# lowmee/xchu_slam

Measured on AMD Instinct MI355X. Metric: NDT scans/sec (120k-pt scan vs 200k-voxel localmap, 30 iters) at 1/2/4/8 GPUs; % HBM BW, higher is better.
Workload: dtype f32 (f64 accumulate)

## Files before the change

xchu_slam_amd/csrc/host_sort.hip:

```cpp
#include "ndt_host.h"

namespace ndt::host {

ndt_status scan_ctx(ndt_ctx* c, Lane L, int nb, ScanCtx* sc) {
    sc->tickets = c->opt.tile_tickets ? 1 : 0;
    if ((size_t)nb > L.s.scan_status.cap) {
        TRY(ensure(c, L.s.scan_status, (size_t)nb));
        HIPCHK(c, hipMemsetAsync(L.s.scan_status.p, 0, L.s.scan_status.cap * sizeof(unsigned long long), L.st));
    }
    if (!L.s.scan_ticket.p) {
        TRY(ensure(c, L.s.scan_ticket, 1));
        HIPCHK(c, hipMemsetAsync(L.s.scan_ticket.p, 0, sizeof(unsigned long long), L.st));
        L.s.scan_tickets = 0;
    }
    sc->status = L.s.scan_status.p;
    sc->ticket = L.s.scan_ticket.p;
    sc->ticket_base = L.s.scan_tickets;
    sc->epoch = ++L.s.scan_epoch;
    sc->nb = nb;
    if (sc->tickets) L.s.scan_tickets += (unsigned long long)nb;
    return NDT_OK;
}

ndt_status enqueue_scan(ndt_ctx* c, Lane L, const int* in, int n_host, const int* n_dev, int* out, int* total_out, GridHeader* herr) {
// ... 17 lines not shown
}

int radix_launch_passes(const ndt_ctx* c) {
    if (c->rerun_full) return 4;
    return c->opt.radix_force > 0 ? std::min(c->opt.radix_force, 4) : c->radix_pred;
}
void note_grid_width(ndt_ctx* c, long long cells, int dense) {
    if (cells <= 0) return;
    const long long top = dense ? cells - 1 : cells;
    int bits = 0;
    while (bits < 31 && (top >> bits) != 0) ++bits;
    c->radix_pred = std::min(4, std::max(1, (bits + 1 + 7) / 8));
}

ndt_status enqueue_bin_and_sort(ndt_ctx* c, Lane L, const float4* pts, int n, int dense, GridHeader* h, float leaf, int layout,
                                int binning, int2* cloud_span, int passes) {
    if (&L.s == &c->s && !cloud_span) c->inc_ok = false;
    const int nb_mm = std::max(1, std::min(ceil_div(n, 4 * kBlock), 1024));
    TRY(ensure(c, L.s.mm, (size_t)nb_mm * 7));
    const int items = radix_items(c, n);
    const int nb_sort = std::max(1, ceil_div(n, kBlock * items));
    const size_t n_kv = cloud_span ? (size_t)n + (size_t)n / 4 : (size_t)n;
    TRY(ensure(c, L.s.k0, n_kv)); TRY(ensure(c, L.s.v0, n_kv)); TRY(ensure(c, L.s.k1, n_kv)); TRY(ensure(c, L.s.v1, n_kv));
    TRY(ensure(c, L.s.radix_aux, kRadixAuxWords));
    TRY(ensure(c, L.s.radix_status, radix_status_words(nb_sort)));
    TRY(ensure(c, L.s.seg_start, (size_t)n + 1));
    hipLaunchKernelGGL(k_minmax, dim3(nb_mm), dim3(kBlock), 0, L.st, pts, n, dense, L.s.mm.p, L.s.radix_aux.p,
                       cloud_span ? c->d_clk.p + 3 : nullptr, nullptr, nullptr, nullptr);
    const int nb_keys = std::max(1, std::min(ceil_div(n, 4 * kBlock), 512));
    hipLaunchKernelGGL(k_keys, dim3(nb_keys), dim3(kBlock), 0, L.st, pts, n, dense, L.s.mm.p, nb_mm, h, leaf, c->prm.min_points_per_voxel,
                       c->prm.min_covar_eigvalue_mult, layout, binning, L.s.k0.p, L.s.v0.p, L.s.radix_aux.p, L.s.radix_status.p,
                       (int)radix_status_words(nb_sort), cloud_span ? c->grid.p : nullptr, (long long)c->grid.cap, cloud_span ? c->table.p : nullptr,
                       1LL << c->max_log2cap, nullptr, 0);
    for (int pass = 0; pass < passes; ++pass)
        launch_radix_pass(c, L, items, nb_sort, L.s.k0.p, L.s.v0.p, L.s.k1.p, L.s.v1.p, n, pass, h, h, passes - 1);
    const int nb_seg = std::max(1, ceil_div(n, kTileKeys));
    ScanCtx sc;
    TRY(scan_ctx(c, L, nb_seg, &sc));
    hipLaunchKernelGGL(k_seg_scan, dim3(nb_seg), dim3(kBlock), 0, L.st, L.s.k0.p, L.s.k1.p, n, h, L.s.seg_start.p, sc);
    if (cloud_span) {
        ScanCtx sc2;
        TRY(scan_ctx(c, L, nb_seg, &sc2));
        hipLaunchKernelGGL(k_cloud_scan, dim3(nb_seg), dim3(kBlock), 0, L.st, L.s.seg_start.p, n, h, cloud_span, sc2, c->max_log2cap);
    }
    return NDT_OK;
}

ndt_status enqueue_downsample_finalize(ndt_ctx* c, Lane L, const GridHeader* h, const float4* in, int n, float4* out) {
    TRY(ensure(c, L.s.sorted_pts, std::max(n, 1)));
    const int nb = std::max(1, std::min(ceil_div(n, 4 * kBlock), 2048));
    hipLaunchKernelGGL(k_sorted_gather, dim3(nb), dim3(kBlock), 0, L.st, in, L.s.v0.p, L.s.v1.p, h, L.s.sorted_pts.p, n);
    hipLaunchKernelGGL(k_downsample_finalize, dim3(std::max(1, ceil_div(n, kBlock))), dim3(kBlock), 0, L.st, L.s.sorted_pts.p,
                       L.s.seg_start.p, h, out);
    HIPCHK(c, hipGetLastError());
    return NDT_OK;
}

}
```

xchu_slam_amd/csrc/host_target.hip:

```cpp
#include "ndt_host.h"

namespace ndt::host {

namespace {

ndt_status grow_grid(ndt_ctx* c) {
    const long long want_cells = std::min<long long>(std::max<long long>(2 * c->grid_cells_seen, 16ll << 20), 1ll << 30);
    if ((long long)c->grid.cap < want_cells) TRY(ensure(c, c->grid, (size_t)want_cells));
    return NDT_OK;
}

ndt_status alloc_cloud_buffers(ndt_ctx* c, size_t max_cloud) {
    TRY(ensure(c, c->recs, max_cloud)); TRY(ensure(c, c->cent, max_cloud)); TRY(ensure(c, c->icovd, max_cloud * 9));
    TRY(ensure(c, c->evals, max_cloud * 3)); TRY(ensure(c, c->cloud_key, max_cloud));
    return NDT_OK;
}

constexpr int kFinalize3WavesMaxPoints = 4 << 20;

ndt_status prepare_target_buffers(ndt_ctx* c, int M, int* nb_cloud) {
    TRY(grow_grid(c));
    const size_t max_cloud = std::max(1, M / std::max(1, c->prm.min_points_per_voxel) + 1);
    TRY(alloc_cloud_buffers(c, max_cloud));
    unsigned l = 6;
    while (l < 30 && (1ull << l) < 4ull * max_cloud) ++l;
    c->max_log2cap = l;
    TRY(ensure(c, c->table, (size_t)1 << l));
    *nb_cloud = std::max(1, ceil_div((long long)max_cloud, kBlock));
    TRY(ensure(c, c->s.cloud_span, (size_t)*nb_cloud * kBlock));
    TRY(ensure(c, c->valid_part, max_cloud / 64 + 1));
    return NDT_OK;
}

ndt_status launch_finalize(ndt_ctx* c, int M, int nb_cloud) {
    auto* fin = M < kFinalize3WavesMaxPoints ? k_leaf_finalize<3> : k_leaf_finalize<2>;
    hipLaunchKernelGGL(fin, dim3(nb_cloud), dim3(kBlock), 0, c->stream.get(), c->target_ptr, c->s.k0.p, c->s.k1.p, c->s.v0.p,
                       c->s.v1.p, c->s.cloud_span.p, c->d_hdr.p, c->recs.p, c->cent.p, c->icovd.p, c->cloud_key.p,
                       c->evals.p, c->grid.p, c->table.p, c->valid_part.p);
    HIPCHK(c, hipGetLastError());
    return NDT_OK;
}

ndt_status enqueue_target_build(ndt_ctx* c) {
    c->inc_ok = false;
    ++c->n_builds_full;
    const int M = c->M;
    int nb_cloud = 0;
    TRY(prepare_target_buffers(c, M, &nb_cloud));
    TRY(enqueue_bin_and_sort(c, main_lane(c), c->target_ptr, M, c->target_dense, c->d_hdr.p, c->prm.resolution, 0, c->prm.precision_mode == 2 ? 1 : 0,
                             c->s.cloud_span.p, radix_launch_passes(c)));
    TRY(launch_finalize(c, M, nb_cloud));
    c->inc_ok = c->prm.precision_mode != 2 && c->target_dense == 1 && M > 0;
    return NDT_OK;
}

ndt_status enqueue_target_append(ndt_ctx* c, int n_old, int n_new, const float4* new_src) {
    const int M = n_old + n_new;
    int nb_cloud = 0;
    TRY(prepare_target_buffers(c, M, &nb_cloud));
    Lane Q{c->stream.get(), c->s_inc};
    float4* copy_to = new_src ? const_cast<float4*>(c->target_ptr) + n_old : nullptr;
    const float4* pts_new = new_src ? new_src : c->target_ptr + n_old;
    const int nq = std::max(n_new, 1);
    const int nb_mm = std::max(1, std::min(ceil_div(nq, 4 * kBlock), 1024));
    TRY(ensure(c, Q.s.mm, (size_t)nb_mm * 7));
    const int items = radix_items(c, nq);
    const int nb_sort = std::max(1, ceil_div(nq, kBlock * items));
    TRY(ensure(c, Q.s.k0, nq)); TRY(ensure(c, Q.s.v0, nq)); TRY(ensure(c, Q.s.k1, nq)); TRY(ensure(c, Q.s.v1, nq));
    TRY(ensure(c, Q.s.radix_aux, kRadixAuxWords));
    TRY(ensure(c, Q.s.radix_status, radix_status_words(nb_sort)));
    TRY(ensure(c, c->s.seg_start, (size_t)M + 1));
    hipLaunchKernelGGL(k_minmax, dim3(nb_mm), dim3(kBlock), 0, c->stream.get(), pts_new, n_new, 1, Q.s.mm.p, Q.s.radix_aux.p, c->d_clk.p + 3,
                       c->d_hdr.p, c->d_hdr_prev.p, copy_to);
    if (c->tgt_ev_valid) HIPCHK(c, hipEventRecord(c->ev_tgt.get(), c->stream.get()));
    const long long clear_words = std::max<long long>((long long)c->grid.cap, 2LL << c->max_log2cap) / 4;
    const int nb_keys = std::max(1, (int)std::min<long long>(std::max<long long>(ceil_div(nq, 4 * kBlock), ceil_div(clear_words, 4LL * kBlock)), 512));
    hipLaunchKernelGGL(k_keys, dim3(nb_keys), dim3(kBlock), 0, c->stream.get(), pts_new, n_new, 1, Q.s.mm.p, nb_mm, c->d_hdr.p, c->prm.resolution,
                       c->prm.min_points_per_voxel, c->prm.min_covar_eigvalue_mult, 0, 0, Q.s.k0.p, Q.s.v0.p, Q.s.radix_aux.p,
                       Q.s.radix_status.p, (int)radix_status_words(nb_sort), c->grid.p, (long long)c->grid.cap, c->table.p, 1LL << c->max_log2cap,
                       c->d_hdr_prev.p, n_old);
    const int passes = radix_launch_passes(c);
    for (int pass = 0; pass < passes; ++pass)
        launch_radix_pass(c, Q, items, nb_sort, Q.s.k0.p, Q.s.v0.p, Q.s.k1.p, Q.s.v1.p, n_new, pass, c->d_hdr.p, c->d_hdr.p, passes - 1);
    hipLaunchKernelGGL(k_merge_append, dim3(std::max(1, ceil_div(M, kMergeTileKeys))), dim3(kBlock), 0, c->stream.get(), c->s.k0.p, c->s.v0.p,
                       c->s.k1.p, c->s.v1.p, c->d_hdr_prev.p, n_old, Q.s.k0.p, Q.s.v0.p, Q.s.k1.p, Q.s.v1.p, n_new, c->d_hdr.p,
                       c->target_ptr);
    const Lane L = main_lane(c);
    const int nb_seg = std::max(1, ceil_div(M, kTileKeys));
    ScanCtx sc, sc2;
    TRY(scan_ctx(c, L, nb_seg, &sc));
    hipLaunchKernelGGL(k_seg_scan, dim3(nb_seg), dim3(kBlock), 0, c->stream.get(), c->s.k0.p, c->s.k1.p, M, c->d_hdr.p, c->s.seg_start.p, sc);
    TRY(scan_ctx(c, L, nb_seg, &sc2));
    hipLaunchKernelGGL(k_cloud_scan, dim3(nb_seg), dim3(kBlock), 0, c->stream.get(), c->s.seg_start.p, M, c->d_hdr.p, c->s.cloud_span.p, sc2,
                       c->max_log2cap);
    TRY(launch_finalize(c, M, nb_cloud));
    return NDT_OK;
}

}

ndt_status build_target(ndt_ctx* c) {
    ++c->tgt_gen;
    c->tgt_ev_valid = c->lanes.fit_tgt_used;
    if (c->tgt_ev_valid) HIPCHK(c, hipEventRecord(c->ev_tgt.get(), c->stream.get()));
    TRY(enqueue_target_build(c));
    c->build_unchecked = true;
    c->built_since_align = true;
    c->grid_valid = true;
    c->fit_valid = false;
    c->grid_res = c->prm.resolution;
// ... 202 lines not shown
```

xchu_slam_amd/csrc/ndt_api.hip:

```cpp
#include "ndt_host.h"

static bool valid_params(const ndt_params* p) {
    return p && p->resolution > 0.f && std::isfinite(p->resolution) && p->max_iter >= 0 && p->search >= 0 && p->search <= 3 &&
           p->min_points_per_voxel >= 1 && p->precision_mode >= 0 && p->precision_mode <= 2;
}

static ndt_status create_buffers(ndt_ctx* c) {
    for (DevBuf<GridHeader>* h : {&c->d_hdr, &c->d_hdr_ds, &c->d_hdr_prev, &c->fe.d_hdr, &c->fit_ix.hdr, &c->fe.sor_ix.hdr}) TRY(ensure(c, *h, 1));
    HIPCHK(c, hipMemset(c->fe.d_hdr.p, 0, sizeof(GridHeader)));
    TRY(make_pinned(c, c->h_hdr, 1, hipHostMallocDefault));
    TRY(ensure(c, c->d_state, 1));
    TRY(ensure(c, c->d_state2, 1));
    TRY(make_pinned(c, c->h_state, 1, hipHostMallocCoherent));
    TRY(make_pinned(c, c->h_rb, 8, hipHostMallocCoherent));
    TRY(ensure(c, c->d_clk, 4));
    TRY(ensure(c, c->d_hist, c->hist_cap));
    TRY(ensure(c, c->d_async, 1));
    TRY(make_pinned(c, c->h_async, 1, hipHostMallocDefault));
    TRY(make_event(c, c->ev_tgt, hipEventDisableTiming));
    std::memset(c->h_state.get(), 0, sizeof(AlignState));
    std::memset(c->h_rb.get(), 0, 8 * sizeof(unsigned long long));
    return NDT_OK;
}

// ... 199 lines not shown
```

xchu_slam_amd/csrc/ndt_host.h:

```cpp
#pragma once
#include <hip/hip_runtime.h>
#include <string>
#include <vector>
#include <cstring>
#include <cstdlib>
#include <cstdio>
#include <algorithm>
#include <cmath>
#include <atomic>
#include <condition_variable>
#include <deque>
#include <functional>
#include <memory>
#include <mutex>
#include <shared_mutex>
#include <thread>

#include "../../include/ndt_hip.h"
#include "ndt_kernels.h"

namespace ndt::host {

constexpr int kTileKeys = kBlock * 16;

// ... 211 lines not shown
    Pinned<AsyncOut> h_async;
    SideLanes lanes;
    Scratch s;
    Scratch s_inc;
    DevBuf<GridHeader> d_hdr_prev;
    bool inc_ok = false;
    int radix_pred = 4;
    bool build_unchecked = false;
    bool rerun_full = false;
    float al_guess[16] = {0};
    int al_berr = 0;
    long long n_builds_full = 0, n_builds_merge = 0, n_builds_rerun = 0, n_rerun_lookback = 0;
    unsigned long long tgt_gen = 0, fit_ix_gen = ~0ull, align_tgt_gen = ~0ull;
    DevBuf<VoxelRec> recs;
    DevBuf<float4> cent;
    DevBuf<double> icovd, evals;
    DevBuf<int> cloud_key;
    DevBuf<int> valid_part;
    DevBuf<int2> table;
    unsigned max_log2cap = 6;
    DevBuf<int> grid;
    long long grid_cells_seen = 0;
    DevBuf<float4> source;
    int N = 0;
    bool has_source = false;
    const float4* src_pend = nullptr;
    DevBuf<float4> source_ord;
    DevBuf<int> ord_k0, ord_v0, ord_k1, ord_v1;
    const float4* pass_src = nullptr;
    FrontEnd fe;
    DevBuf<AlignState> d_state;
    DevBuf<AlignState> d_state2;
    int lead = 0, lead_par = 0;
    bool no_lead = false;
    Pinned<AlignState> h_state;
    Pinned<unsigned long long[]> h_rb;
// ... 88 lines not shown
    h->opt = c->opt;
    h->opt.tile_tickets = sticky || c->opt.tile_tickets;
}

inline ndt_status set_dev(ndt_ctx* c) {
    HIPCHK(c, hipSetDevice(c->device));
    return NDT_OK;
}

inline ndt_status need_target_and_source(ndt_ctx* c) {
    if (!c->has_target) return fail(c, NDT_ENOTARGET, "no input target");
    if (!c->has_source || c->N == 0) return fail(c, NDT_ENOSOURCE, "no input source");
    return NDT_OK;
}

ndt_status scan_ctx(ndt_ctx* c, Lane L, int nb, ScanCtx* sc);
ndt_status enqueue_scan(ndt_ctx* c, Lane L, const int* in, int n_host, const int* n_dev, int* out, int* total_out, GridHeader* herr);
int radix_items(const ndt_ctx* c, int n);
size_t radix_status_words(int nb);
void launch_radix_pass(const ndt_ctx* c, Lane L, int items, int nb, int* k0, int* v0, int* k1, int* v1, int n, int pass,
                       const GridHeader* h, GridHeader* herr, int last_pass = 3);
int radix_launch_passes(const ndt_ctx* c);
void note_grid_width(ndt_ctx* c, long long cells, int dense);
ndt_status enqueue_bin_and_sort(ndt_ctx* c, Lane L, const float4* pts, int n, int dense, GridHeader* h, float leaf, int layout = 0,
                                int binning = 0, int2* cloud_span = nullptr, int passes = 4);
ndt_status enqueue_downsample_finalize(ndt_ctx* c, Lane L, const GridHeader* h, const float4* in, int n, float4* out);
ndt_status build_target(ndt_ctx* c);
ndt_status rerun_build(ndt_ctx* c, int berr);
ndt_status settle_build(ndt_ctx* c);
ndt_status upload_points(ndt_ctx* c, DevBuf<float4>& dst, const float* xyz, size_t n, size_t stride_bytes);
void invalidate_graph(ndt_ctx* c);
ndt_status copy16(ndt_ctx* c, hipStream_t stream, void* dst, const void* src, size_t bytes);
ndt_status flush_source(ndt_ctx* c);
ndt_status capture_graph(ndt_ctx* c, const char* end_what, const std::function<ndt_status()>& body, GraphExec* out);
ndt_status main_after_fit(ndt_ctx* c, bool source);
ndt_status enqueue_nn_index(ndt_ctx* c, Lane L, const float4* pts, int n, int dense, float cell, NNIndex& ix, bool want_idx = false);
ndt_status ensure_fit_index(ndt_ctx* c);
ndt_status reserve_slots(ndt_ctx* c, SlotArrays& a, size_t size, size_t need, std::initializer_list<size_t> slot_bytes, const char* what);

}
// ... 1 lines not shown
```

xchu_slam_amd/csrc/ndt_kernels.h:

```cpp
#pragma once
#include <hip/hip_runtime.h>
#include "ndt_types.h"
#include "ndt_linalg.h"
#include "ndt_icp.h"
#include "ndt_sc.h"
#include "ndt_isc.h"
#include "ndt_pgo.h"

namespace ndt {
__global__ void k_minmax(const float4*, int, int, float*, int*, unsigned long long*, const GridHeader*, GridHeader*, float4*);
__global__ void k_keys(const float4*, int, int, const float*, int, GridHeader*, float, int, double, int, int, int*, int*, int*, unsigned*, int,
                       int*, long long, int2*, long long, const GridHeader*, int);
__global__ void k_merge_append(int*, int*, int*, int*, const GridHeader*, int, const int*, const int*, const int*, const int*, int,
                               GridHeader*, const float4*);
template <int ITEMS>
__global__ void k_radix_onesweep(int*, int*, int*, int*, int, int, const GridHeader*, int*, unsigned*, int, GridHeader*, int, int);
__global__ void k_scan_onepass(const int*, int, const int*, int*, int*, ScanCtx, GridHeader*);
__global__ void k_seg_scan(const int*, const int*, int, GridHeader*, int*, ScanCtx);
__global__ void k_cloud_scan(const int*, int, GridHeader*, int2*, ScanCtx, unsigned);

template <int WAVES>
__global__ void k_leaf_finalize(const float4*, const int*, const int*, const int*, const int*, const int2*, GridHeader*,
                                VoxelRec*, float4*, double*, int*, double*, int*, int2*, int*);
__global__ void k_sorted_gather(const float4*, const int*, const int*, const GridHeader*, float4*, int);
__global__ void k_src_keys(const float4*, int, Mat4f, const GridHeader*, int*, int*, int*, unsigned*, int);
__global__ void k_src_gather(const float4*, const int*, const int*, const GridHeader*, float4*, int);
__global__ void k_crop_flags(const float4*, int, double, double, int*);
__global__ void k_compact4(const float4*, const int*, const int*, int, float4*);
template <int C>
__global__ void k_sor_knn(const float4*, int, int, const GridHeader*, const int*, const int*, const float4*, float*);
__global__ void k_sor_stats(const float*, int, double, double*);
__global__ void k_sor_keep(const float*, int, const double*, int*);
__global__ void k_ror_keep(const float4*, int, double, int, const GridHeader*, const int*, const int*, const float4*, int*);
__global__ void k_downsample_finalize(const float4*, const int*, const GridHeader*, float4*);
__global__ void k_fit_gather(const float4*, const int*, const int*, const int*, const int*, const int*, int, const GridHeader*, float4*,
                             int*, int*, int*);
__global__ void k_icp_pass(float4*, int, IcpState*, const GridHeader*, const int*, const int*, const float4*, const int*, int*, float*,
                           double*, unsigned*, IcpRecordDev*);
// ... 37 lines not shown
```

xchu_slam_amd/csrc/voxel_build.hip:

```cpp
#include "ndt_device.h"
#include "ndt_kernels.h"

namespace ndt {

constexpr int kTileItems = 16;
constexpr int kTile = kBlock * kTileItems;
constexpr int kRadixAux = kRadixAuxWords;

__global__ __launch_bounds__(kBlock) void k_minmax(const float4* __restrict__ pts, int n, int is_dense, float* __restrict__ part,
                                                   int* __restrict__ radix_aux, unsigned long long* __restrict__ clk_start,
                                                   const GridHeader* __restrict__ hdr_cur, GridHeader* __restrict__ hdr_save,
                                                   float4* __restrict__ copy_to) {
    if (clk_start && blockIdx.x == 0 && threadIdx.x == 0) *clk_start = __builtin_amdgcn_s_memrealtime();
    if (blockIdx.x == 0) {
        for (int i = threadIdx.x; i < kRadixAux; i += kBlock) radix_aux[i] = 0;
        if (hdr_save) {
            static_assert(sizeof(GridHeader) % 4 == 0 && sizeof(GridHeader) / 4 <= kBlock, "header copy: one word per thread");
            if (threadIdx.x < sizeof(GridHeader) / 4)
                reinterpret_cast<int*>(hdr_save)[threadIdx.x] = reinterpret_cast<const int*>(hdr_cur)[threadIdx.x];
        }
    }
    float mn[3] = {FLT_MAX, FLT_MAX, FLT_MAX}, mx[3] = {-FLT_MAX, -FLT_MAX, -FLT_MAX};
    int cnt = 0;
    const int stride = gridDim.x * kBlock;
    for (int i0 = blockIdx.x * kBlock + threadIdx.x; i0 < n; i0 += 4 * stride) {
        float4 q[4];
#pragma unroll
        for (int u = 0; u < 4; ++u) q[u] = i0 + u * stride < n ? pts[i0 + u * stride] : make_float4(0.f, 0.f, 0.f, 0.f);
// ... 169 lines not shown
                                                 const GridHeader* __restrict__ fold, int val_base) {
    for (int i = blockIdx.x * kBlock + threadIdx.x; i < status_words; i += gridDim.x * kBlock) status[i] = 0u;
    __shared__ GridHeader s_h;
    __shared__ float s_red[kBlock][7];
    header_body(part, nb_mm, &s_h, leaf, min_pts, eig_mult, is_dense, layout, binning, s_red, fold);
    __syncthreads();
    const bool lookup = grid != nullptr && !s_h.empty;
    const bool dense = lookup && s_h.cells > 0 && s_h.cells <= grid_cap;
    if (blockIdx.x == 0 && threadIdx.x == 0) {
        GridHeader g = s_h;
        g.dense = dense ? 1 : 0;
        *hout = g;
    }
    const GridHeader* h = &s_h;
    if (h->empty) return;
    if (lookup) {
        const long long words = dense ? s_h.cells : 2 * table_slots;
        const int4 fill = dense ? make_int4(-1, -1, -1, -1) : make_int4(kEmptyKey, 0, kEmptyKey, 0);
        int4* dst = dense ? reinterpret_cast<int4*>(grid) : reinterpret_cast<int4*>(table);
        const long long m4 = words / 4;
        for (long long i = (long long)blockIdx.x * kBlock + threadIdx.x; i < m4; i += (long long)gridDim.x * kBlock) dst[i] = fill;
        if (blockIdx.x == 0 && threadIdx.x < (int)(words - 4 * m4)) {
            int* w = dense ? grid : reinterpret_cast<int*>(table);
            w[4 * m4 + threadIdx.x] = (threadIdx.x & 1) && !dense ? 0 : -1;
        }
    }
    const int passes = (h->key_bits + 7) / 8;
    __shared__ int cnt[4][256];
    for (int q = 0; q < 4; ++q) cnt[q][threadIdx.x] = 0;
    __syncthreads();
    const int stride = gridDim.x * kBlock;
    for (int i0 = blockIdx.x * kBlock + threadIdx.x; i0 < n; i0 += 4 * stride) {
        float4 p[4];
#pragma unroll
        for (int u = 0; u < 4; ++u) p[u] = i0 + u * stride < n ? pts[i0 + u * stride] : make_float4(0.f, 0.f, 0.f, 0.f);
#pragma unroll
        for (int u = 0; u < 4; ++u) {
            const int i = i0 + u * stride;
            if (i >= n) break;
            const int key = voxel_key(p[u], is_dense, h);
// ... 513 lines not shown
            if (key != sentinel && (i == 0 || prev != key)) { heads |= 1u << q; ++sum; }
            prev = key;
        }
    }
    int total;
    int ex = tile_scan(sc, sum, h, &s_tile, &s_excl, lds, tile, &total);
#pragma unroll
    for (int q = 0; q < kTileItems; ++q)
        if (heads & (1u << q)) seg_start[ex++] = base + q;
    if (tile == sc.nb - 1 && threadIdx.x == 0) {
        h->n_leaves = total;
        seg_start[total] = empty ? 0 : h->n_points;
    }
}

__global__ __launch_bounds__(kBlock) void k_cloud_scan(const int* __restrict__ seg_start, int n, GridHeader* __restrict__ h,
                                                       int2* __restrict__ cloud_span, ScanCtx sc, unsigned max_log2cap) {
    __shared__ int s_tile, s_excl, lds[4];
    __shared__ int s_seg[kStageWords];
    const int tile = take_ticket(sc, &s_tile);
    const int nl = h->empty ? 0 : h->n_leaves;
    const int last = nl > 0 ? (nl - 1) / kTile : 0;
    if (tile > last) return;
    const int base = tile * kTile + threadIdx.x * kTileItems;
    const int minp = h->min_points;
    unsigned fl = 0;
    int sum = 0;
    stage_tile<1>(seg_start, (long long)tile * kTile, nl + 1, 0, s_seg);
#pragma unroll
    for (int q = 0; q < kTileItems; ++q) {
        const int s = base + q;
        if (s >= nl) break;
        const int p = threadIdx.x * kTileItems + q;
        if (s_seg[st_idx(p + 1)] - s_seg[st_idx(p)] >= minp) { fl |= 1u << q; ++sum; }
    }
    int total;
    int ex = tile_scan(sc, sum, h, &s_tile, &s_excl, lds, tile, &total);
#pragma unroll
    for (int q = 0; q < kTileItems; ++q)
        if (fl & (1u << q)) {
            const int p = threadIdx.x * kTileItems + q;
            cloud_span[ex++] = make_int2(s_seg[st_idx(p)], s_seg[st_idx(p + 1)]);
        }
    if (tile == last && threadIdx.x == 0) {
        h->n_cloud = total;
        unsigned l = 6;
        while (l < max_log2cap && (1LL << l) < 4LL * (long long)total) ++l;
        h->log2cap = l;
        if (total == 0) h->empty = 1;
    }
}






constexpr int kGather = 8;
__device__ __forceinline__ bool leaf_stats(const float4* __restrict__ pts, const int* __restrict__ idx, int b, int e, int ci, int key,
                                           const GridHeader* __restrict__ h, VoxelRec* __restrict__ recs, float4* __restrict__ cent,
                                           double* __restrict__ icovd, int* __restrict__ cloud_key, double* __restrict__ evals_out) {
    const int n = e - b;
    double sum[3] = {0.0, 0.0, 0.0};
    double cov[9] = {1.0, 0.0, 0.0, 0.0, 1.0, 0.0, 0.0, 0.0, 1.0};
    float cen[3] = {0.f, 0.f, 0.f};
    int ix[kGather];
#pragma unroll
    for (int k = 0; k < kGather; ++k) ix[k] = (b + k < e) ? idx[b + k] : -1;
    for (int j0 = b; j0 < e; j0 += kGather) {
        float4 q[kGather];
#pragma unroll
        for (int k = 0; k < kGather; ++k) q[k] = ix[k] >= 0 ? pts[ix[k]] : make_float4(0.f, 0.f, 0.f, 0.f);
#pragma unroll
        for (int k = 0; k < kGather; ++k) ix[k] = (j0 + kGather + k < e) ? idx[j0 + kGather + k] : -1;
#pragma unroll
        for (int k = 0; k < kGather; ++k) {
// ... 46 lines not shown
        inverse3<double>(cov, icov);
        double mxv = -HUGE_VAL, mnv = HUGE_VAL;
        for (int k = 0; k < 9; ++k) { mxv = fmax(mxv, icov[k]); mnv = fmin(mnv, icov[k]); }
        if (!h->binning && (mxv == HUGE_VAL || mnv == -HUGE_VAL)) rejected = true;
    }
    VoxelRec rec;
    for (int a = 0; a < 3; ++a) rec.mean[a] = mean[a];
    for (int r = 0; r < 3; ++r)
        for (int c = 0; c < 3; ++c) rec.icov[r * 3 + c] = (float)icov[r + 3 * c];
    rec.npts = rejected ? -1 : n;
    recs[ci] = rec;
    cent[ci] = make_float4(cen[0], cen[1], cen[2], 0.f);
    for (int r = 0; r < 3; ++r)
        for (int c = 0; c < 3; ++c) icovd[(size_t)ci * 9 + r * 3 + c] = icov[r + 3 * c];
    cloud_key[ci] = key;
    for (int a = 0; a < 3; ++a) evals_out[(size_t)ci * 3 + a] = ev[a];
    return rejected;
}

template <int WAVES>
__global__ __launch_bounds__(kBlock) __attribute__((amdgpu_waves_per_eu(WAVES))) void k_leaf_finalize(const float4* __restrict__ pts, const int* __restrict__ k0,
                                                          const int* __restrict__ k1, const int* __restrict__ v0,
                                                          const int* __restrict__ v1, const int2* __restrict__ cloud_span,
                                                          GridHeader* __restrict__ h,
                                                          VoxelRec* __restrict__ recs, float4* __restrict__ cent,
                                                          double* __restrict__ icovd, int* __restrict__ cloud_key,
                                                          double* __restrict__ evals_out, int* __restrict__ grid,
                                                          int2* __restrict__ table, int* __restrict__ valid_part) {
    const int ci = blockIdx.x * kBlock + threadIdx.x;
    const int2 be = cloud_span[ci];
    if (ci >= h->n_cloud) return;
    const int* keys = sorted_buf(h, k0, k1);
    const int* vals = sorted_buf(h, v0, v1);
    const int b = be.x, e = be.y;
    const int key = keys[b];
    const bool rejected = leaf_stats(pts, vals, b, e, ci, key, h, recs, cent, icovd, cloud_key, evals_out);
    const unsigned long long ok = __ballot(!rejected);
    if ((threadIdx.x & 63) == 0) valid_part[ci >> 6] = (int)__popcll(ok);
    const int val = ci | (rejected ? kRejectBit : 0);
    if (h->dense) {
        if (key >= 0 && (long long)key < h->cells) grid[key] = val;
        return;
    }
    const unsigned log2cap = h->log2cap;
    const unsigned mask = (1u << log2cap) - 1u;
    unsigned slot = hash_slot(key, log2cap);
    const unsigned long long empty = (unsigned long long)(unsigned)kEmptyKey;
    const unsigned long long mine = ((unsigned long long)(unsigned)val << 32) | (unsigned)key;
    unsigned long long* t = reinterpret_cast<unsigned long long*>(table);
    for (;;) {
        const unsigned long long prev = atomicCAS(&t[slot], empty, mine);
// ... 17 lines not shown
    for (int i0 = blockIdx.x * (kBlock * U) + threadIdx.x; i0 < m; i0 += gridDim.x * (kBlock * U)) {
        int v[U];
#pragma unroll
        for (int u = 0; u < U; ++u) v[u] = i0 + u * kBlock < m ? vals[i0 + u * kBlock] : -1;
        float4 q[U];
#pragma unroll
        for (int u = 0; u < U; ++u) q[u] = v[u] >= 0 ? pts[v[u]] : make_float4(0.f, 0.f, 0.f, 0.f);
#pragma unroll
        for (int u = 0; u < U; ++u)
            if (v[u] >= 0) sorted[i0 + u * kBlock] = q[u];
    }
}

#define NDT_FIN_INST(W)                                                                                                   \
    template __global__ void k_leaf_finalize<W>(const float4*, const int*, const int*, const int*, const int*, const int2*, \
                                                GridHeader*, VoxelRec*, float4*, double*, int*, double*, int*, int2*, int*);
NDT_FIN_INST(2)
NDT_FIN_INST(3)
#undef NDT_FIN_INST

__global__ __launch_bounds__(kBlock) void k_src_keys(const float4* __restrict__ src, int n, Mat4f Tm, const GridHeader* __restrict__ h,
                                                     int* __restrict__ keys, int* __restrict__ vals, int* __restrict__ radix_aux,
                                                     unsigned* __restrict__ status, int status_words) {
    for (int i = blockIdx.x * kBlock + threadIdx.x; i < status_words; i += gridDim.x * kBlock) status[i] = 0u;
    if (h->empty) return;
    const int passes = (h->key_bits + 7) / 8;
    const float* T = Tm.m;
    __shared__ int cnt[4][256];
    for (int q = 0; q < 4; ++q) cnt[q][threadIdx.x] = 0;
    __syncthreads();
    for (int i = blockIdx.x * kBlock + threadIdx.x; i < n; i += gridDim.x * kBlock) {
// ... 397 lines not shown
```

Measured before the change: 1306.

## Fuse segment and cloud scans, clear dense grid sparsely, drop unused eigenvalue output

```diff
diff --git a/xchu_slam_amd/csrc/host_sort.hip b/xchu_slam_amd/csrc/host_sort.hip
--- a/xchu_slam_amd/csrc/host_sort.hip
+++ b/xchu_slam_amd/csrc/host_sort.hip
@@ -2,10 +2,10 @@
 
 namespace ndt::host {
 
-ndt_status scan_ctx(ndt_ctx* c, Lane L, int nb, ScanCtx* sc) {
+ndt_status scan_ctx(ndt_ctx* c, Lane L, int nb, ScanCtx* sc, int sums) {
     sc->tickets = c->opt.tile_tickets ? 1 : 0;
-    if ((size_t)nb > L.s.scan_status.cap) {
-        TRY(ensure(c, L.s.scan_status, (size_t)nb));
+    if ((size_t)nb * sums > L.s.scan_status.cap) {
+        TRY(ensure(c, L.s.scan_status, (size_t)nb * sums));
         HIPCHK(c, hipMemsetAsync(L.s.scan_status.p, 0, L.s.scan_status.cap * sizeof(unsigned long long), L.st));
     }
     if (!L.s.scan_ticket.p) {
@@ -55,7 +55,7 @@
 }
 
 ndt_status enqueue_bin_and_sort(ndt_ctx* c, Lane L, const float4* pts, int n, int dense, GridHeader* h, float leaf, int layout,
-                                int binning, int2* cloud_span, int passes) {
+                                int binning, int2* cloud_span, int passes, bool unset_grid) {
     if (&L.s == &c->s && !cloud_span) c->inc_ok = false;
     const int nb_mm = std::max(1, std::min(ceil_div(n, 4 * kBlock), 1024));
     TRY(ensure(c, L.s.mm, (size_t)nb_mm * 7));
@@ -67,7 +67,8 @@
     TRY(ensure(c, L.s.radix_status, radix_status_words(nb_sort)));
     TRY(ensure(c, L.s.seg_start, (size_t)n + 1));
     hipLaunchKernelGGL(k_minmax, dim3(nb_mm), dim3(kBlock), 0, L.st, pts, n, dense, L.s.mm.p, L.s.radix_aux.p,
-                       cloud_span ? c->d_clk.p + 3 : nullptr, nullptr, nullptr, nullptr);
+                       cloud_span ? c->d_clk.p + 3 : nullptr, h, nullptr, nullptr, cloud_span && unset_grid ? c->grid.p : nullptr,
+                       (long long)c->grid.cap, c->cloud_key.p, (int)c->cloud_key.cap);
     const int nb_keys = std::max(1, std::min(ceil_div(n, 4 * kBlock), 512));
     hipLaunchKernelGGL(k_keys, dim3(nb_keys), dim3(kBlock), 0, L.st, pts, n, dense, L.s.mm.p, nb_mm, h, leaf, c->prm.min_points_per_voxel,
                        c->prm.min_covar_eigvalue_mult, layout, binning, L.s.k0.p, L.s.v0.p, L.s.radix_aux.p, L.s.radix_status.p,
@@ -75,15 +76,21 @@
                        1LL << c->max_log2cap, nullptr, 0);
     for (int pass = 0; pass < passes; ++pass)
         launch_radix_pass(c, L, items, nb_sort, L.s.k0.p, L.s.v0.p, L.s.k1.p, L.s.v1.p, n, pass, h, h, passes - 1);
+    if (cloud_span) return enqueue_seg_cloud_scan(c, L, n, h, cloud_span);
     const int nb_seg = std::max(1, ceil_div(n, kTileKeys));
     ScanCtx sc;
     TRY(scan_ctx(c, L, nb_seg, &sc));
     hipLaunchKernelGGL(k_seg_scan, dim3(nb_seg), dim3(kBlock), 0, L.st, L.s.k0.p, L.s.k1.p, n, h, L.s.seg_start.p, sc);
-    if (cloud_span) {
-        ScanCtx sc2;
-        TRY(scan_ctx(c, L, nb_seg, &sc2));
-        hipLaunchKernelGGL(k_cloud_scan, dim3(nb_seg), dim3(kBlock), 0, L.st, L.s.seg_start.p, n, h, cloud_span, sc2, c->max_log2cap);
-    }
+    return NDT_OK;
+}
+
+ndt_status enqueue_seg_cloud_scan(ndt_ctx* c, Lane L, int n, GridHeader* h, int2* cloud_span) {
+    const int nb_seg = std::max(1, ceil_div(n, kTileKeys));
+    const int cloud_cap = std::max(1, n / std::max(1, c->prm.min_points_per_voxel) + 1);
+    ScanCtx sc;
+    TRY(scan_ctx(c, L, nb_seg, &sc, 2));
+    hipLaunchKernelGGL(k_seg_cloud_scan, dim3(nb_seg), dim3(kBlock), 0, L.st, L.s.k0.p, L.s.k1.p, n, h, L.s.seg_start.p, cloud_span,
+                       cloud_cap, sc, c->max_log2cap);
     return NDT_OK;
 }
 
diff --git a/xchu_slam_amd/csrc/host_target.hip b/xchu_slam_amd/csrc/host_target.hip
--- a/xchu_slam_amd/csrc/host_target.hip
+++ b/xchu_slam_amd/csrc/host_target.hip
@@ -12,16 +12,20 @@
 
 ndt_status alloc_cloud_buffers(ndt_ctx* c, size_t max_cloud) {
     TRY(ensure(c, c->recs, max_cloud)); TRY(ensure(c, c->cent, max_cloud)); TRY(ensure(c, c->icovd, max_cloud * 9));
-    TRY(ensure(c, c->evals, max_cloud * 3)); TRY(ensure(c, c->cloud_key, max_cloud));
+    TRY(ensure(c, c->cloud_key, max_cloud));
     return NDT_OK;
 }
 
 constexpr int kFinalize3WavesMaxPoints = 4 << 20;
 
-ndt_status prepare_target_buffers(ndt_ctx* c, int M, int* nb_cloud) {
+ndt_status prepare_target_buffers(ndt_ctx* c, int M, int* nb_cloud, bool* unset_grid) {
+    const size_t grid_cap = c->grid.cap, key_cap = c->cloud_key.cap;
     TRY(grow_grid(c));
     const size_t max_cloud = std::max(1, M / std::max(1, c->prm.min_points_per_voxel) + 1);
     TRY(alloc_cloud_buffers(c, max_cloud));
+    *unset_grid = c->grid_clean && !c->rerun_full && c->grid.cap == grid_cap && c->cloud_key.cap == key_cap;
+    c->grid_clean = false;
+    if (!*unset_grid) HIPCHK(c, hipMemsetAsync(c->grid.p, 0xff, c->grid.cap * sizeof(int), c->stream.get()));
     unsigned l = 6;
     while (l < 30 && (1ull << l) < 4ull * max_cloud) ++l;
     c->max_log2cap = l;
@@ -36,7 +40,7 @@
     auto* fin = M < kFinalize3WavesMaxPoints ? k_leaf_finalize<3> : k_leaf_finalize<2>;
     hipLaunchKernelGGL(fin, dim3(nb_cloud), dim3(kBlock), 0, c->stream.get(), c->target_ptr, c->s.k0.p, c->s.k1.p, c->s.v0.p,
                        c->s.v1.p, c->s.cloud_span.p, c->d_hdr.p, c->recs.p, c->cent.p, c->icovd.p, c->cloud_key.p,
-                       c->evals.p, c->grid.p, c->table.p, c->valid_part.p);
+                       c->grid.p, c->table.p, c->valid_part.p);
     HIPCHK(c, hipGetLastError());
     return NDT_OK;
 }
@@ -46,10 +50,12 @@
     ++c->n_builds_full;
     const int M = c->M;
     int nb_cloud = 0;
-    TRY(prepare_target_buffers(c, M, &nb_cloud));
+    bool unset_grid = false;
+    TRY(prepare_target_buffers(c, M, &nb_cloud, &unset_grid));
     TRY(enqueue_bin_and_sort(c, main_lane(c), c->target_ptr, M, c->target_dense, c->d_hdr.p, c->prm.resolution, 0, c->prm.precision_mode == 2 ? 1 : 0,
-                             c->s.cloud_span.p, radix_launch_passes(c)));
+                             c->s.cloud_span.p, radix_launch_passes(c), unset_grid));
     TRY(launch_finalize(c, M, nb_cloud));
+    c->grid_clean = true;
     c->inc_ok = c->prm.precision_mode != 2 && c->target_dense == 1 && M > 0;
     return NDT_OK;
 }
@@ -57,12 +63,13 @@
 ndt_status enqueue_target_append(ndt_ctx* c, int n_old, int n_new, const float4* new_src) {
     const int M = n_old + n_new;
     int nb_cloud = 0;
-    TRY(prepare_target_buffers(c, M, &nb_cloud));
+    bool unset_grid = false;
+    TRY(prepare_target_buffers(c, M, &nb_cloud, &unset_grid));
     Lane Q{c->stream.get(), c->s_inc};
     float4* copy_to = new_src ? const_cast<float4*>(c->target_ptr) + n_old : nullptr;
     const float4* pts_new = new_src ? new_src : c->target_ptr + n_old;
     const int nq = std::max(n_new, 1);
-    const int nb_mm = std::max(1, std::min(ceil_div(nq, 4 * kBlock), 1024));
+    const int nb_mm = std::max(1, std::min(std::max(ceil_div(nq, 4 * kBlock), unset_grid ? ceil_div((long long)c->cloud_key.cap, 4 * kBlock) : 0), 1024));
     TRY(ensure(c, Q.s.mm, (size_t)nb_mm * 7));
     const int items = radix_items(c, nq);
     const int nb_sort = std::max(1, ceil_div(nq, kBlock * items));
@@ -71,9 +78,10 @@
     TRY(ensure(c, Q.s.radix_status, radix_status_words(nb_sort)));
     TRY(ensure(c, c->s.seg_start, (size_t)M + 1));
     hipLaunchKernelGGL(k_minmax, dim3(nb_mm), dim3(kBlock), 0, c->stream.get(), pts_new, n_new, 1, Q.s.mm.p, Q.s.radix_aux.p, c->d_clk.p + 3,
-                       c->d_hdr.p, c->d_hdr_prev.p, copy_to);
+                       c->d_hdr.p, c->d_hdr_prev.p, copy_to, unset_grid ? c->grid.p : nullptr, (long long)c->grid.cap, c->cloud_key.p,
+                       (int)c->cloud_key.cap);
     if (c->tgt_ev_valid) HIPCHK(c, hipEventRecord(c->ev_tgt.get(), c->stream.get()));
-    const long long clear_words = std::max<long long>((long long)c->grid.cap, 2LL << c->max_log2cap) / 4;
+    const long long clear_words = (2LL << c->max_log2cap) / 4;
     const int nb_keys = std::max(1, (int)std::min<long long>(std::max<long long>(ceil_div(nq, 4 * kBlock), ceil_div(clear_words, 4LL * kBlock)), 512));
     hipLaunchKernelGGL(k_keys, dim3(nb_keys), dim3(kBlock), 0, c->stream.get(), pts_new, n_new, 1, Q.s.mm.p, nb_mm, c->d_hdr.p, c->prm.resolution,
                        c->prm.min_points_per_voxel, c->prm.min_covar_eigvalue_mult, 0, 0, Q.s.k0.p, Q.s.v0.p, Q.s.radix_aux.p,
@@ -85,15 +93,9 @@
     hipLaunchKernelGGL(k_merge_append, dim3(std::max(1, ceil_div(M, kMergeTileKeys))), dim3(kBlock), 0, c->stream.get(), c->s.k0.p, c->s.v0.p,
                        c->s.k1.p, c->s.v1.p, c->d_hdr_prev.p, n_old, Q.s.k0.p, Q.s.v0.p, Q.s.k1.p, Q.s.v1.p, n_new, c->d_hdr.p,
                        c->target_ptr);
-    const Lane L = main_lane(c);
-    const int nb_seg = std::max(1, ceil_div(M, kTileKeys));
-    ScanCtx sc, sc2;
-    TRY(scan_ctx(c, L, nb_seg, &sc));
-    hipLaunchKernelGGL(k_seg_scan, dim3(nb_seg), dim3(kBlock), 0, c->stream.get(), c->s.k0.p, c->s.k1.p, M, c->d_hdr.p, c->s.seg_start.p, sc);
-    TRY(scan_ctx(c, L, nb_seg, &sc2));
-    hipLaunchKernelGGL(k_cloud_scan, dim3(nb_seg), dim3(kBlock), 0, c->stream.get(), c->s.seg_start.p, M, c->d_hdr.p, c->s.cloud_span.p, sc2,
-                       c->max_log2cap);
+    TRY(enqueue_seg_cloud_scan(c, main_lane(c), M, c->d_hdr.p, c->s.cloud_span.p));
     TRY(launch_finalize(c, M, nb_cloud));
+    c->grid_clean = true;
     return NDT_OK;
 }
 
diff --git a/xchu_slam_amd/csrc/ndt_api.hip b/xchu_slam_amd/csrc/ndt_api.hip
--- a/xchu_slam_amd/csrc/ndt_api.hip
+++ b/xchu_slam_amd/csrc/ndt_api.hip
@@ -8,6 +8,7 @@
 static ndt_status create_buffers(ndt_ctx* c) {
     for (DevBuf<GridHeader>* h : {&c->d_hdr, &c->d_hdr_ds, &c->d_hdr_prev, &c->fe.d_hdr, &c->fit_ix.hdr, &c->fe.sor_ix.hdr}) TRY(ensure(c, *h, 1));
     HIPCHK(c, hipMemset(c->fe.d_hdr.p, 0, sizeof(GridHeader)));
+    HIPCHK(c, hipMemset(c->d_hdr.p, 0, sizeof(GridHeader)));
     TRY(make_pinned(c, c->h_hdr, 1, hipHostMallocDefault));
     TRY(ensure(c, c->d_state, 1));
     TRY(ensure(c, c->d_state2, 1));
diff --git a/xchu_slam_amd/csrc/ndt_host.h b/xchu_slam_amd/csrc/ndt_host.h
--- a/xchu_slam_amd/csrc/ndt_host.h
+++ b/xchu_slam_amd/csrc/ndt_host.h
@@ -249,12 +249,13 @@
     unsigned long long tgt_gen = 0, fit_ix_gen = ~0ull, align_tgt_gen = ~0ull;
     DevBuf<VoxelRec> recs;
     DevBuf<float4> cent;
-    DevBuf<double> icovd, evals;
+    DevBuf<double> icovd;
     DevBuf<int> cloud_key;
     DevBuf<int> valid_part;
     DevBuf<int2> table;
     unsigned max_log2cap = 6;
     DevBuf<int> grid;
+    bool grid_clean = false;
     long long grid_cells_seen = 0;
     DevBuf<float4> source;
     int N = 0;
@@ -373,7 +374,7 @@
     return NDT_OK;
 }
 
-ndt_status scan_ctx(ndt_ctx* c, Lane L, int nb, ScanCtx* sc);
+ndt_status scan_ctx(ndt_ctx* c, Lane L, int nb, ScanCtx* sc, int sums = 1);
 ndt_status enqueue_scan(ndt_ctx* c, Lane L, const int* in, int n_host, const int* n_dev, int* out, int* total_out, GridHeader* herr);
 int radix_items(const ndt_ctx* c, int n);
 size_t radix_status_words(int nb);
@@ -382,7 +383,8 @@
 int radix_launch_passes(const ndt_ctx* c);
 void note_grid_width(ndt_ctx* c, long long cells, int dense);
 ndt_status enqueue_bin_and_sort(ndt_ctx* c, Lane L, const float4* pts, int n, int dense, GridHeader* h, float leaf, int layout = 0,
-                                int binning = 0, int2* cloud_span = nullptr, int passes = 4);
+                                int binning = 0, int2* cloud_span = nullptr, int passes = 4, bool unset_grid = false);
+ndt_status enqueue_seg_cloud_scan(ndt_ctx* c, Lane L, int n, GridHeader* h, int2* cloud_span);
 ndt_status enqueue_downsample_finalize(ndt_ctx* c, Lane L, const GridHeader* h, const float4* in, int n, float4* out);
 ndt_status build_target(ndt_ctx* c);
 ndt_status rerun_build(ndt_ctx* c, int berr);
diff --git a/xchu_slam_amd/csrc/ndt_kernels.h b/xchu_slam_amd/csrc/ndt_kernels.h
--- a/xchu_slam_amd/csrc/ndt_kernels.h
+++ b/xchu_slam_amd/csrc/ndt_kernels.h
@@ -8,7 +8,8 @@
 #include "ndt_pgo.h"
 
 namespace ndt {
-__global__ void k_minmax(const float4*, int, int, float*, int*, unsigned long long*, const GridHeader*, GridHeader*, float4*);
+__global__ void k_minmax(const float4*, int, int, float*, int*, unsigned long long*, const GridHeader*, GridHeader*, float4*, int*,
+                         long long, const int*, int);
 __global__ void k_keys(const float4*, int, int, const float*, int, GridHeader*, float, int, double, int, int, int*, int*, int*, unsigned*, int,
                        int*, long long, int2*, long long, const GridHeader*, int);
 __global__ void k_merge_append(int*, int*, int*, int*, const GridHeader*, int, const int*, const int*, const int*, const int*, int,
@@ -17,11 +18,11 @@
 __global__ void k_radix_onesweep(int*, int*, int*, int*, int, int, const GridHeader*, int*, unsigned*, int, GridHeader*, int, int);
 __global__ void k_scan_onepass(const int*, int, const int*, int*, int*, ScanCtx, GridHeader*);
 __global__ void k_seg_scan(const int*, const int*, int, GridHeader*, int*, ScanCtx);
-__global__ void k_cloud_scan(const int*, int, GridHeader*, int2*, ScanCtx, unsigned);
+__global__ void k_seg_cloud_scan(const int*, const int*, int, GridHeader*, int*, int2*, int, ScanCtx, unsigned);
 
 template <int WAVES>
 __global__ void k_leaf_finalize(const float4*, const int*, const int*, const int*, const int*, const int2*, GridHeader*,
-                                VoxelRec*, float4*, double*, int*, double*, int*, int2*, int*);
+                                VoxelRec*, float4*, double*, int*, int*, int2*, int*);
 __global__ void k_sorted_gather(const float4*, const int*, const int*, const GridHeader*, float4*, int);
 __global__ void k_src_keys(const float4*, int, Mat4f, const GridHeader*, int*, int*, int*, unsigned*, int);
 __global__ void k_src_gather(const float4*, const int*, const int*, const GridHeader*, float4*, int);
diff --git a/xchu_slam_amd/csrc/voxel_build.hip b/xchu_slam_amd/csrc/voxel_build.hip
--- a/xchu_slam_amd/csrc/voxel_build.hip
+++ b/xchu_slam_amd/csrc/voxel_build.hip
@@ -10,8 +10,21 @@
 __global__ __launch_bounds__(kBlock) void k_minmax(const float4* __restrict__ pts, int n, int is_dense, float* __restrict__ part,
                                                    int* __restrict__ radix_aux, unsigned long long* __restrict__ clk_start,
                                                    const GridHeader* __restrict__ hdr_cur, GridHeader* __restrict__ hdr_save,
-                                                   float4* __restrict__ copy_to) {
+                                                   float4* __restrict__ copy_to, int* __restrict__ grid, long long grid_cap,
+                                                   const int* __restrict__ cloud_key, int cloud_cap) {
     if (clk_start && blockIdx.x == 0 && threadIdx.x == 0) *clk_start = __builtin_amdgcn_s_memrealtime();
+    if (grid && hdr_cur->dense) {
+        const int nc = min(hdr_cur->n_cloud, cloud_cap);
+        const int stride = gridDim.x * kBlock;
+        for (int i0 = blockIdx.x * kBlock + threadIdx.x; i0 < nc; i0 += 4 * stride) {
+            int key[4];
+#pragma unroll
+            for (int u = 0; u < 4; ++u) key[u] = i0 + u * stride < nc ? cloud_key[i0 + u * stride] : -1;
+#pragma unroll
+            for (int u = 0; u < 4; ++u)
+                if (key[u] >= 0 && (long long)key[u] < grid_cap) grid[key[u]] = -1;
+        }
+    }
     if (blockIdx.x == 0) {
         for (int i = threadIdx.x; i < kRadixAux; i += kBlock) radix_aux[i] = 0;
         if (hdr_save) {
@@ -211,16 +224,11 @@
     }
     const GridHeader* h = &s_h;
     if (h->empty) return;
-    if (lookup) {
-        const long long words = dense ? s_h.cells : 2 * table_slots;
-        const int4 fill = dense ? make_int4(-1, -1, -1, -1) : make_int4(kEmptyKey, 0, kEmptyKey, 0);
-        int4* dst = dense ? reinterpret_cast<int4*>(grid) : reinterpret_cast<int4*>(table);
-        const long long m4 = words / 4;
+    if (lookup && !dense) {
+        const int4 fill = make_int4(kEmptyKey, 0, kEmptyKey, 0);
+        int4* dst = reinterpret_cast<int4*>(table);
+        const long long m4 = table_slots / 2;
         for (long long i = (long long)blockIdx.x * kBlock + threadIdx.x; i < m4; i += (long long)gridDim.x * kBlock) dst[i] = fill;
-        if (blockIdx.x == 0 && threadIdx.x < (int)(words - 4 * m4)) {
-            int* w = dense ? grid : reinterpret_cast<int*>(table);
-            w[4 * m4 + threadIdx.x] = (threadIdx.x & 1) && !dense ? 0 : -1;
-        }
     }
     const int passes = (h->key_bits + 7) / 8;
     __shared__ int cnt[4][256];
@@ -764,40 +772,177 @@
     }
 }
 
-__global__ __launch_bounds__(kBlock) void k_cloud_scan(const int* __restrict__ seg_start, int n, GridHeader* __restrict__ h,
-                                                       int2* __restrict__ cloud_span, ScanCtx sc, unsigned max_log2cap) {
-    __shared__ int s_tile, s_excl, lds[4];
-    __shared__ int s_seg[kStageWords];
+__device__ void scan_lookback2(unsigned long long* __restrict__ st_a, unsigned long long* __restrict__ st_b, int tile, int tot_a,
+                               int tot_b, unsigned epoch, GridHeader* __restrict__ herr, int* excl_a, int* excl_b) {
+    const int lane = threadIdx.x & 63;
+    const unsigned long long tag = (unsigned long long)epoch << 32;
+    if (lane == 0) {
+        const unsigned long long f = tag | (tile == 0 ? kScanPre : kScanAgg);
+        __hip_atomic_store(&st_a[tile], f | (unsigned long long)tot_a, __ATOMIC_RELAXED, __HIP_MEMORY_SCOPE_AGENT);
+        __hip_atomic_store(&st_b[tile], f | (unsigned long long)tot_b, __ATOMIC_RELAXED, __HIP_MEMORY_SCOPE_AGENT);
+    }
+    long long ea = 0, eb = 0;
+    int t = tile - 1;
+    int spin = 0;
+    while (t >= 0) {
+        const int tt = t - lane;
+        unsigned long long wa = 0, wb = 0;
+        bool ready = true;
+        if (tt >= 0) {
+            wa = __hip_atomic_load(&st_a[tt], __ATOMIC_RELAXED, __HIP_MEMORY_SCOPE_AGENT);
+            wb = __hip_atomic_load(&st_b[tt], __ATOMIC_RELAXED, __HIP_MEMORY_SCOPE_AGENT);
+            const unsigned long long fa = wa & (kScanAgg | kScanPre);
+            ready = (wa >> 32) == epoch && (wb >> 32) == epoch && fa != 0 && fa == (wb & (kScanAgg | kScanPre));
+        }
+        const bool pre = tt >= 0 && ready && (wa & kScanPre);
+        const unsigned long long pre_mask = __ballot(pre);
+        const int stop = pre_mask ? (__ffsll((long long)pre_mask) - 1) : 63;
+        const unsigned long long need = (stop == 63) ? ~0ull : ((2ull << stop) - 1);
+        const unsigned long long not_ready = __ballot(!ready) & need;
+        if (not_ready) {
+            if (++spin > kSpinLimit) { if (lane == 0) atomicOr(&herr->pad[0], kBuildErrLookback); break; }
+            __builtin_amdgcn_s_sleep(1);
+            continue;
+        }
+        const bool take = tt >= 0 && lane <= stop;
+        long long va = take ? (long long)(wa & kScanVal) : 0, vb = take ? (long long)(wb & kScanVal) : 0;
+        for (int m = 32; m > 0; m >>= 1) { va += __shfl_xor(va, m, 64); vb += __shfl_xor(vb, m, 64); }
+        ea += va;
+        eb += vb;
+        if (pre_mask) break;
+        t -= 64;
+    }
+    if (lane == 0 && tile > 0) {
+        __hip_atomic_store(&st_a[tile], tag | kScanPre | ((unsigned long long)(ea + tot_a) & kScanVal), __ATOMIC_RELAXED,
+                           __HIP_MEMORY_SCOPE_AGENT);
+        __hip_atomic_store(&st_b[tile], tag | kScanPre | ((unsigned long long)(eb + tot_b) & kScanVal), __ATOMIC_RELAXED,
+                           __HIP_MEMORY_SCOPE_AGENT);
+    }
+    *excl_a = (int)ea;
+    *excl_b = (int)eb;
+}
+
+__global__ __launch_bounds__(kBlock) void k_seg_cloud_scan(const int* __restrict__ k0, const int* __restrict__ k1, int n,
+                                                           GridHeader* __restrict__ h, int* __restrict__ seg_start,
+                                                           int2* __restrict__ cloud_span, int cloud_cap, ScanCtx sc,
+                                                           unsigned max_log2cap) {
+    __shared__ int s_tile, s_sent, s_excl[2], lds[4];
+    __shared__ int s_k[kStageWords];
+    static_assert(kStageWords >= kTile + 1, "s_pos in s_k");
+    int* s_pos = s_k;
     const int tile = take_ticket(sc, &s_tile);
-    const int nl = h->empty ? 0 : h->n_leaves;
-    const int last = nl > 0 ? (nl - 1) / kTile : 0;
-    if (tile > last) return;
-    const int base = tile * kTile + threadIdx.x * kTileItems;
+    const bool empty = h->empty != 0;
+    const int* k = sorted_buf(h, k0, k1);
+    const int sentinel = h->sentinel;
     const int minp = h->min_points;
+    const int t0 = tile * kTile, t1 = min(t0 + kTile, n);
+    const int base = t0 + threadIdx.x * kTileItems;
+    unsigned heads = 0;
+    int sum = 0;
+    if (threadIdx.x == 0) s_sent = -1;
+    int next_key = 0;
+    if (!empty) {
+        if (threadIdx.x < 64 && t1 + (int)threadIdx.x < n) next_key = k[t1 + threadIdx.x];
+        stage_tile<1>(k, (long long)t0 - 1, n, 0, s_k);
+        int prev = s_k[st_idx(threadIdx.x * kTileItems)];
+#pragma unroll
+        for (int q = 0; q < kTileItems; ++q) {
+            const int i = base + q;
+            if (i >= n) break;
+            const int key = s_k[st_idx(threadIdx.x * kTileItems + q + 1)];
+            if (i == 0 || prev != key) {
+                if (key != sentinel) { heads |= 1u << q; ++sum; }
+                else s_sent = i;
+            }
+            prev = key;
+        }
+    }
+    const int last_key = empty ? 0 : s_k[st_idx(t1 - t0)];
+    int ltot;
+    const int lex = block_exclusive_scan(sum, lds, &ltot);
+    {
+        int r = lex;
+#pragma unroll
+        for (int q = 0; q < kTileItems; ++q)
+            if (heads & (1u << q)) s_pos[r++] = base + q;
+    }
+    __syncthreads();
+    if (threadIdx.x < 64 && ltot > 0) {
+        const int lane = threadIdx.x;
+        int end = s_sent;
+        if (end < 0) {
+            end = n;
+            if (t1 < n) {
+                const unsigned long long diff = __ballot(t1 + lane >= n || next_key != last_key);
+                if (diff) {
+                    end = min(t1 + __ffsll((long long)diff) - 1, n);
+                } else {
+                    int lo = t1 + 64, hi = n;
+                    while (lo < hi) {
+                        const int step = (hi - lo + 63) / 64;
+                        const long long m = (long long)lo + (long long)lane * step;
+                        const bool probe = m < hi;
+                        const bool same = probe && k[m] == last_key;
+                        const unsigned long long probed = __ballot(probe);
+                        const unsigned long long fls = __ballot(probe && !same);
+                        if (fls == 0ull) {
+                            lo = lo + (63 - __clzll((long long)probed)) * step + 1;
+                        } else {
+                            const int f = __ffsll((long long)fls) - 1;
+                            const int nlo = f == 0 ? lo : lo + (f - 1) * step + 1;
+                            hi = lo + f * step;
+                            lo = nlo;
+                        }
+                    }
+                    end = lo;
+                }
+            }
+        }
+        if (lane == 0) s_pos[ltot] = end;
+    }
+    __syncthreads();
     unsigned fl = 0;
-    int sum = 0;
-    stage_tile<1>(seg_start, (long long)tile * kTile, nl + 1, 0, s_seg);
-#pragma unroll
-    for (int q = 0; q < kTileItems; ++q) {
-        const int s = base + q;
-        if (s >= nl) break;
-        const int p = threadIdx.x * kTileItems + q;
-        if (s_seg[st_idx(p + 1)] - s_seg[st_idx(p)] >= minp) { fl |= 1u << q; ++sum; }
-    }
-    int total;
-    int ex = tile_scan(sc, sum, h, &s_tile, &s_excl, lds, tile, &total);
-#pragma unroll
-    for (int q = 0; q < kTileItems; ++q)
-        if (fl & (1u << q)) {
-            const int p = threadIdx.x * kTileItems + q;
-            cloud_span[ex++] = make_int2(s_seg[st_idx(p)], s_seg[st_idx(p + 1)]);
-        }
-    if (tile == last && threadIdx.x == 0) {
-        h->n_cloud = total;
+    int csum = 0;
+    {
+        int r = lex;
+#pragma unroll
+        for (int q = 0; q < kTileItems; ++q)
+            if (heads & (1u << q)) {
+                if (s_pos[r + 1] - s_pos[r] >= minp) { fl |= 1u << q; ++csum; }
+                ++r;
+            }
+    }
+    int ctot;
+    const int cex = block_exclusive_scan(csum, lds, &ctot);
+    if (threadIdx.x < 64) {
+        int ea, eb;
+        scan_lookback2(sc.status, sc.status + sc.nb, tile, ltot, ctot, sc.epoch, h, &ea, &eb);
+        if (threadIdx.x == 0) { s_excl[0] = ea; s_excl[1] = eb; }
+    }
+    __syncthreads();
+    {
+        int r = lex, cw = s_excl[1] + cex;
+        int* seg_out = seg_start + s_excl[0];
+#pragma unroll
+        for (int q = 0; q < kTileItems; ++q)
+            if (heads & (1u << q)) {
+                seg_out[r] = s_pos[r];
+                if (fl & (1u << q)) {
+                    if (cw < cloud_cap) cloud_span[cw] = make_int2(s_pos[r], s_pos[r + 1]);
+                    ++cw;
+                }
+                ++r;
+            }
+    }
+    if (tile == sc.nb - 1 && threadIdx.x == 0) {
+        const int leaves = s_excl[0] + ltot, cloud = min(s_excl[1] + ctot, cloud_cap);
+        h->n_leaves = leaves;
+        seg_start[leaves] = empty ? 0 : h->n_points;
+        h->n_cloud = cloud;
         unsigned l = 6;
-        while (l < max_log2cap && (1LL << l) < 4LL * (long long)total) ++l;
+        while (l < max_log2cap && (1LL << l) < 4LL * (long long)cloud) ++l;
         h->log2cap = l;
-        if (total == 0) h->empty = 1;
+        if (cloud == 0) h->empty = 1;
     }
 }
 
@@ -809,7 +954,7 @@
 constexpr int kGather = 8;
 __device__ __forceinline__ bool leaf_stats(const float4* __restrict__ pts, const int* __restrict__ idx, int b, int e, int ci, int key,
                                            const GridHeader* __restrict__ h, VoxelRec* __restrict__ recs, float4* __restrict__ cent,
-                                           double* __restrict__ icovd, int* __restrict__ cloud_key, double* __restrict__ evals_out) {
+                                           double* __restrict__ icovd, int* __restrict__ cloud_key) {
     const int n = e - b;
     double sum[3] = {0.0, 0.0, 0.0};
     double cov[9] = {1.0, 0.0, 0.0, 0.0, 1.0, 0.0, 0.0, 0.0, 1.0};
@@ -886,7 +1031,6 @@
     for (int r = 0; r < 3; ++r)
         for (int c = 0; c < 3; ++c) icovd[(size_t)ci * 9 + r * 3 + c] = icov[r + 3 * c];
     cloud_key[ci] = key;
-    for (int a = 0; a < 3; ++a) evals_out[(size_t)ci * 3 + a] = ev[a];
     return rejected;
 }
 
@@ -897,8 +1041,8 @@
                                                           GridHeader* __restrict__ h,
                                                           VoxelRec* __restrict__ recs, float4* __restrict__ cent,
                                                           double* __restrict__ icovd, int* __restrict__ cloud_key,
-                                                          double* __restrict__ evals_out, int* __restrict__ grid,
-                                                          int2* __restrict__ table, int* __restrict__ valid_part) {
+                                                          int* __restrict__ grid, int2* __restrict__ table,
+                                                          int* __restrict__ valid_part) {
     const int ci = blockIdx.x * kBlock + threadIdx.x;
     const int2 be = cloud_span[ci];
     if (ci >= h->n_cloud) return;
@@ -906,7 +1050,7 @@
     const int* vals = sorted_buf(h, v0, v1);
     const int b = be.x, e = be.y;
     const int key = keys[b];
-    const bool rejected = leaf_stats(pts, vals, b, e, ci, key, h, recs, cent, icovd, cloud_key, evals_out);
+    const bool rejected = leaf_stats(pts, vals, b, e, ci, key, h, recs, cent, icovd, cloud_key);
     const unsigned long long ok = __ballot(!rejected);
     if ((threadIdx.x & 63) == 0) valid_part[ci >> 6] = (int)__popcll(ok);
     const int val = ci | (rejected ? kRejectBit : 0);
@@ -954,7 +1098,7 @@
 
 #define NDT_FIN_INST(W)                                                                                                   \
     template __global__ void k_leaf_finalize<W>(const float4*, const int*, const int*, const int*, const int*, const int2*, \
-                                                GridHeader*, VoxelRec*, float4*, double*, int*, double*, int*, int2*, int*);
+                                                GridHeader*, VoxelRec*, float4*, double*, int*, int*, int2*, int*);
 NDT_FIN_INST(2)
 NDT_FIN_INST(3)
 #undef NDT_FIN_INST
```

Result: no change. 1310 (median of 6 runs) (+0.3%).
